# boqian-li/ETCH

Measured on AMD Instinct MI355X. Metric: scans/s (5k pts, eq-net + 50-iter SMPL fit), higher is better.
Workload: dtype f32 (matrix operands: 2 x fp16 planes per fp32 value, fp32 accumulate)

## Files before the change

### etch_amd/csrc/index_ops.hip

```cpp
#include "common.h"
#include <cmath>
#include <cstdio>

template <int WAVES>
__global__ void __launch_bounds__(WAVES * 64) ball_query_kernel(int n, int m, float radius2, int nsample,
                                                               const float* __restrict__ new_xyz,
                                                               const float* __restrict__ xyz, int* __restrict__ idx) {
    extern __shared__ __attribute__((aligned(16))) int smem_i[];
    const int lane = threadIdx.x & 63, wave = threadIdx.x >> 6;
    const int b = blockIdx.y;
    const float* X = xyz + (size_t)b * 3 * n;
    const float* Q = new_xyz + (size_t)b * 3 * m;
    int* row = smem_i + wave * nsample;
    for (int j = blockIdx.x * WAVES + wave; j < m; j += gridDim.x * WAVES) {
        const float qx = Q[j], qy = Q[m + j], qz = Q[2 * m + j];
        int cnt = 0;
        for (int k0 = 0; k0 < n && cnt < nsample; k0 += 64) {
            const int k = k0 + lane;
            bool in = false;
            if (k < n) {
                float d2 = etch_sqdist(qx, qy, qz, X[k], X[n + k], X[2 * n + k]);
                in = d2 < radius2;
            }
            const unsigned long long mask = __ballot(in);
// ... 455 lines not shown
        if (lane == 0) {
            for (int i = nsample - 1; i > 0; i--) {
                float tf = hd[0]; hd[0] = hd[i]; hd[i] = tf;
                int ti = hi[0]; hi[0] = hi[i]; hi[i] = ti;
                int root = 0, child = 1;
                while (child < i) {
                    if (child + 1 < i && hd[child + 1] > hd[child]) child++;
                    if (hd[root] > hd[child]) break;
                    const float tf2 = hd[root]; hd[root] = hd[child]; hd[child] = tf2;
                    const int ti2 = hi[root]; hi[root] = hi[child]; hi[child] = ti2;
                    root = child; child = root * 2 + 1;
                }
            }
        }
        __builtin_amdgcn_wave_barrier();
        for (int i = lane; i < nsample; i += 64) {
            idx[(size_t)q * nsample + i] = hi[i];
            const float d = hd[i];
            dist2[(size_t)q * nsample + i] = write_sqrt ? sqrtf(d) : d;
        }
        __builtin_amdgcn_wave_barrier();
}

__global__ void __launch_bounds__(KNNW_WAVES * 64) knn_wave_kernel(int nsample, int nseg, const float* __restrict__ xyz,
                                                                    const float* __restrict__ new_xyz, const int* __restrict__ offset,
                                                                    const int* __restrict__ new_offset, int m_total, int* __restrict__ idx,
                                                                    float* __restrict__ dist2, int write_sqrt) {
    extern __shared__ __attribute__((aligned(16))) float smem_f[];
    const int lane = threadIdx.x & 63, wave = threadIdx.x >> 6;
    float* hd = smem_f + wave * 2 * nsample;
    int* hi = (int*)(hd + nsample);
    float* cand_d = smem_f + KNNW_WAVES * 2 * nsample + wave * 128;
    int* cand_i = (int*)(cand_d + 64);
    for (int q = blockIdx.x * KNNW_WAVES + wave; q < m_total; q += gridDim.x * KNNW_WAVES) {
        int seg = 0;
        while (seg < nseg - 1 && q >= new_offset[seg]) ++seg;
        const int start = seg == 0 ? 0 : offset[seg - 1], end = offset[seg];
        if (nsample > 16) {
            knn_literal_query(q, start, end, nsample, lane, xyz, new_xyz, hd, hi, cand_d, cand_i, idx, dist2, write_sqrt);
            continue;
        }
        const float qx = new_xyz[(size_t)q * 3], qy = new_xyz[(size_t)q * 3 + 1], qz = new_xyz[(size_t)q * 3 + 2];
        float bd = 1e10f;
        int bi = start;
        float top = 1e10f;
        bool ambiguous = false;
        for (int k0 = start; k0 < end; k0 += 64) {
            const int k = k0 + lane;
            float d2 = 3e38f;
            if (k < end) d2 = etch_sqdist(qx, qy, qz, xyz[(size_t)k * 3], xyz[(size_t)k * 3 + 1], xyz[(size_t)k * 3 + 2]);
            unsigned long long mask = __ballot(d2 < top);
            while (mask) {
                const int e = __builtin_ctzll(mask);
                mask &= mask - 1ull;
                const float cd = __int_as_float(__builtin_amdgcn_readlane(__float_as_int(d2), e));
                if (cd < top) {
                    if (nsample > 1) {
                        const float t2 = __int_as_float(__builtin_amdgcn_readlane(__float_as_int(bd), nsample - 2));
                        if (t2 == top && __builtin_amdgcn_readlane(bi, nsample - 1) != __builtin_amdgcn_readlane(bi, nsample - 2)) ambiguous = true;
                    }
                    const int pos = __popcll(__ballot(lane < nsample && bd <= cd));
                    const float pd = __int_as_float(__builtin_amdgcn_update_dpp(0, __float_as_int(bd), 0x111, 0xf, 0xf, true));
                    const int pi = __builtin_amdgcn_update_dpp(0, bi, 0x111, 0xf, 0xf, true);
                    if (lane == pos) { bd = cd; bi = k0 + e; }
                    else if (lane > pos) { bd = pd; bi = pi; }
                    top = __int_as_float(__builtin_amdgcn_readlane(__float_as_int(bd), nsample - 1));
                }
            }
        }
        const float prev = __int_as_float(__builtin_amdgcn_update_dpp(0, __float_as_int(bd), 0x111, 0xf, 0xf, true));
        const int previ = __builtin_amdgcn_update_dpp(0, bi, 0x111, 0xf, 0xf, true);
        const bool tie = lane > 0 && lane < nsample && bd == prev && bi != previ;
        if (ambiguous || __ballot(tie) != 0ull) {
            knn_literal_query(q, start, end, nsample, lane, xyz, new_xyz, hd, hi, cand_d, cand_i, idx, dist2, write_sqrt);
            continue;
        }
        if (lane < nsample) {
            idx[(size_t)q * nsample + lane] = bi;
            dist2[(size_t)q * nsample + lane] = write_sqrt ? sqrtf(bd) : bd;
        }
    }
}

static inline int ilog2_floor_host(int v) { int b = 0; while ((1 << (b + 1)) <= v) ++b; return b; }

static int opt_n_threads_host(int work_size) {
    const int pow_2 = (int)(std::log((double)work_size) / std::log(2.0));
    int v = 1 << pow_2;
    if (v > 1024) v = 1024;
    if (v < 1) v = 1;
    return v;
}

static int g_fps_fast = 1;

static int launch_fps2(int nseg0, int nseg1, int n_max, const FpsProb& p0, const FpsProb& p1, hipStream_t st) {
    const int bs = opt_n_threads_host(n_max);
    const int bits = ilog2_floor_host(bs);
    const bool fits_lds = (size_t)3 * n_max * sizeof(float) <= 62 * 1024;
    const int nseg = nseg0 + nseg1;
#define FPS_CASE(T, P, R, C, COND)                                                                                     \
    if (n_max <= T * P && (COND)) {                                                                                    \
        const int use_lds = !C && fits_lds ? n_max : 0;                                                                \
        if (R && C && T == 1024 && bs == T && g_fps_fast)      \
            hipLaunchKernelGGL((fps_kernel<T, P, R, C, (R && C && T == 1024)>), dim3(nseg), dim3(T), (size_t)3 * use_lds * sizeof(float), st,   \
                               use_lds, p0, p1, nseg0, bs, bits);                                                      \
        else                                                                                                           \
            hipLaunchKernelGGL((fps_kernel<T, P, R, C>), dim3(nseg), dim3(T), (size_t)3 * use_lds * sizeof(float), st, \
                               use_lds, p0, p1, nseg0, bs, bits);                                                      \
        ETCH_RETURN_IF_LAUNCH_FAILED();                                                                                \
        return ETCH_OK;                                                                                                \
    }
    FPS_CASE(64, 1, true, false, true) FPS_CASE(64, 4, true, false, true) FPS_CASE(256, 2, true, false, true) FPS_CASE(256, 8, true, false, true)
    FPS_CASE(1024, 4, true, false, true) FPS_CASE(1024, 8, true, false, fits_lds) FPS_CASE(1024, 8, true, true, true)
    FPS_CASE(1024, 12, true, true, true) FPS_CASE(1024, 20, true, true, true) FPS_CASE(1024, 32, false, false, true)
#undef FPS_CASE
    return ETCH_EUNSUPPORTED;
}

static int launch_fps(int nseg, int n_max, const float* xyz, long cs, long ps, long bstride, int n_fixed, int m_fixed,
                      const int* offset, const int* new_offset, int skip_origin, int* idx, hipStream_t st) {
    const FpsProb p = {xyz, cs, ps, bstride, n_fixed, m_fixed, offset, new_offset, skip_origin, idx};
    return launch_fps2(nseg, 0, n_max, p, p, st);
}

static unsigned g_fps_spin_limit = 1u << 22;
static int g_fps_drop_group = -1;

static int launch_fps_split(int nseg, int n_max, int G, const float* xyz, long cs, long ps, long bstride, int n_fixed, int m_fixed, const int* offset,
                            const int* new_offset, int skip_origin, int* idx, void* workspace, hipStream_t st) {
    if (G < 2 || G > 8 || !workspace) return ETCH_EINVAL;
    const int bs = opt_n_threads_host(n_max);
    const int bits = ilog2_floor_host(bs);
    const int chunks = (n_max + 1023) / 1024, need = (chunks + G - 1) / G;
    const size_t bytes = 64 + (size_t)nseg * 2 * G * 64;
    hipError_t e = hipMemsetAsync(workspace, 0, bytes, st);
    if (e != hipSuccess) return (int)e;
#define FPS_SPLIT_CASE(P)                                                                                                                  \
    if (need <= P) {                                                                                                                       \
        hipLaunchKernelGGL((fps_split_kernel<P>), dim3(nseg * G), dim3(1024), 0, st, G, xyz, cs, ps, bstride, n_fixed, m_fixed, offset,    \
                           new_offset, bs, bits, skip_origin, g_fps_spin_limit, g_fps_drop_group, (unsigned long long*)workspace, idx);    \
        ETCH_RETURN_IF_LAUNCH_FAILED();                                                                                                    \
        return ETCH_OK;                                                                                                                    \
    }
    FPS_SPLIT_CASE(2) FPS_SPLIT_CASE(3) FPS_SPLIT_CASE(4) FPS_SPLIT_CASE(5) FPS_SPLIT_CASE(6) FPS_SPLIT_CASE(8)
#undef FPS_SPLIT_CASE
    return ETCH_EUNSUPPORTED;
}

extern "C" {

int etch_fps_split_workspace_bytes(int nseg, int G) { return nseg > 0 && G > 0 ? 64 + nseg * 2 * G * 64 : 64; }

int etch_furthest_point_sampling_split(int b, int n, int m, const float* xyz, int* idx, int G, void* workspace, void* stream) {
    if (b <= 0 || m <= 0) return ETCH_OK;
    if (n <= 0) return ETCH_EINVAL;
    return launch_fps_split(b, n, G, xyz, (long)n, 1, (long)3 * n, n, m, nullptr, nullptr, 1, idx, workspace, (hipStream_t)stream);
}

int etch_furthestsampling_split(int b, int n_max, const float* xyz, const int* offset, const int* new_offset, int* idx, int G, void* workspace,
                                void* stream) {
    if (b <= 0) return ETCH_OK;
    if (n_max <= 0) return ETCH_EINVAL;
    return launch_fps_split(b, n_max, G, xyz, 1, 3, 0, 0, 0, offset, new_offset, 0, idx, workspace, (hipStream_t)stream);
}

// ... 34 lines not shown

int etch_furthest_point_sampling(int b, int n, int m, const float* xyz, int* idx, void* stream) {
    if (b <= 0 || m <= 0) return ETCH_OK;
    if (n <= 0) return ETCH_EINVAL;
    return launch_fps(b, n, xyz, (long)n, 1, (long)3 * n, n, m, nullptr, nullptr, 1, idx, (hipStream_t)stream);
}

int etch_furthestsampling(int b, int n_max, const float* xyz, const int* offset, const int* new_offset, int* idx,
                          void* stream) {
    if (b <= 0) return ETCH_OK;
    if (n_max <= 0) return ETCH_EINVAL;
    return launch_fps(b, n_max, xyz, 1, 3, 0, 0, 0, offset, new_offset, 0, idx, (hipStream_t)stream);
}

int etch_fps_pair(int b, int n, int m, const float* xyz_b3n, int* idx_a, const float* xyz_packed, const int* offset, const int* new_offset, int* idx_b,
                  void* stream) {
    if (b <= 0) return ETCH_OK;
    if (n <= 0 || m <= 0 || !xyz_b3n || !xyz_packed || !offset || !new_offset || !idx_a || !idx_b) return ETCH_EINVAL;
    const FpsProb p0 = {xyz_b3n, (long)n, 1, (long)3 * n, n, m, nullptr, nullptr, 1, idx_a};
    const FpsProb p1 = {xyz_packed, 1, 3, 0, 0, 0, offset, new_offset, 0, idx_b};
    return launch_fps2(b, b, n, p0, p1, (hipStream_t)stream);
}

int etch_gather_points(int b, int c, int n, int m, const float* points, const int* idx, float* out, void* stream) {
    if (b <= 0 || m <= 0 || c <= 0) return ETCH_OK;
    int gx = (m + 255) / 256;
    if (gx > 8192) gx = 8192;
    hipLaunchKernelGGL(gather_points_kernel, dim3(gx, b), dim3(256), 0, (hipStream_t)stream, c, n, m, points, idx, out);
    ETCH_RETURN_IF_LAUNCH_FAILED();
    return ETCH_OK;
}

int etch_gather_points_backward(int b, int c, int n, int m, const float* grad_out, const int* idx, float* grad_points, void* stream) {
    if (b <= 0 || n <= 0 || c <= 0) return ETCH_OK;
    if (m < 0) return ETCH_EINVAL;
    int gx = (n + 255) / 256;
    if (gx > 8192) gx = 8192;
    hipLaunchKernelGGL(gather_points_backward_kernel, dim3(gx, b), dim3(256), 0, (hipStream_t)stream, c, n, m, grad_out, idx, grad_points);
    ETCH_RETURN_IF_LAUNCH_FAILED();
    return ETCH_OK;
}

int etch_knnquery(int b, int m_max, int m_total, int nsample, const float* xyz, const float* new_xyz, const int* offset,
                  const int* new_offset, int* idx, float* dist, int write_sqrt, void* stream) {
    if (b <= 0 || m_max <= 0) return ETCH_OK;
    if (nsample <= 0) return ETCH_EINVAL;
    if (m_total > 0) {
        if (nsample > 100) return ETCH_EUNSUPPORTED;
        const size_t lds = (size_t)(KNNW_WAVES * 2 * nsample + KNNW_WAVES * 128) * 4;
        long blocks = ((long)m_total + KNNW_WAVES - 1) / KNNW_WAVES;
        if (blocks > 256 * 64) blocks = 256 * 64;
        hipLaunchKernelGGL(knn_wave_kernel, dim3((unsigned)blocks), dim3(KNNW_WAVES * 64), lds, (hipStream_t)stream, nsample, b, xyz,
                           new_xyz, offset, new_offset, m_total, idx, dist, write_sqrt);
        ETCH_RETURN_IF_LAUNCH_FAILED();
        return ETCH_OK;
    }
    if (nsample > 28) return ETCH_EUNSUPPORTED;
    const size_t lds = (size_t)(3 * KNN_TILE + 2 * nsample * KNN_THREADS) * 4;
    hipLaunchKernelGGL(knn_kernel, dim3((m_max + KNN_THREADS - 1) / KNN_THREADS, b), dim3(KNN_THREADS), lds,
                       (hipStream_t)stream, nsample, xyz, new_xyz, offset, new_offset, idx, dist, write_sqrt);
    ETCH_RETURN_IF_LAUNCH_FAILED();
    return ETCH_OK;
}

int etch_knnquery_dev_bounded(int m, int nsample, int nseg, const float* xyz, const float* new_xyz, const int* offset, const int* new_offset,
                              int* idx, float* dist, int write_sqrt, void* stream) {
    if (m <= 0) return ETCH_OK;
    if (nsample <= 0 || nseg <= 0) return ETCH_EINVAL;
    if (nsample > 100) return ETCH_EUNSUPPORTED;
    const size_t lds = (size_t)(KNNW_WAVES * 2 * nsample + KNNW_WAVES * 128) * 4;
    long blocks = ((long)m + KNNW_WAVES - 1) / KNNW_WAVES;
    if (blocks > 256 * 64) blocks = 256 * 64;
    hipLaunchKernelGGL(knn_wave_kernel, dim3((unsigned)blocks), dim3(KNNW_WAVES * 64), lds, (hipStream_t)stream, nsample, nseg, xyz,
                       new_xyz, offset, new_offset, m, idx, dist, write_sqrt);
    ETCH_RETURN_IF_LAUNCH_FAILED();
    return ETCH_OK;
}

int etch_knnquery_dev(int m, int nsample, const float* xyz, const float* new_xyz, const int* offset, const int* new_offset, int* idx,
                      float* dist, int write_sqrt, void* stream) {
    return etch_knnquery_dev_bounded(m, nsample, 0x7fffffff, xyz, new_xyz, offset, new_offset, idx, dist, write_sqrt, stream);
}

static void report_launcher(const char* name, int rc) {
    if (rc != ETCH_OK) fprintf(stderr, "Error: %s failed (%d%s%s)\n", name, rc, rc > 0 ? ": " : "", rc > 0 ? hipGetErrorString((hipError_t)rc) : "");
}

void knnquery_cuda_launcher(int m, int nsample, const float* xyz, const float* new_xyz, const int* offset, const int* new_offset, int* idx,
                            float* dist2) {
    report_launcher("knnquery_cuda_launcher", etch_knnquery_dev(m, nsample, xyz, new_xyz, offset, new_offset, idx, dist2, 0, nullptr));
}

void furthestsampling_cuda_launcher(int b, int n, const float* xyz, const int* offset, const int* new_offset, float* tmp, int* idx) {
    (void)tmp;
    report_launcher("furthestsampling_cuda_launcher", etch_furthestsampling(b, n, xyz, offset, new_offset, idx, nullptr));
}

void ball_query_cuda_launcher(int b, int n, int m, float radius, int nsample, const float* new_xyz, const float* xyz, int* idx) {
    report_launcher("ball_query_cuda_launcher", etch_ball_query(b, n, m, radius, nsample, new_xyz, xyz, idx, nullptr));
}

void furthest_point_sampling_cuda_launcher(int b, int n, int m, const float* dataset, float* temp, int* idxs) {
    (void)temp;
    report_launcher("furthest_point_sampling_cuda_launcher", etch_furthest_point_sampling(b, n, m, dataset, idxs, nullptr));
}

void gather_points_forward_cuda_launcher(int b, int c, int n, int m, const float* points, const int* idx, float* out) {
    report_launcher("gather_points_forward_cuda_launcher", etch_gather_points(b, c, n, m, points, idx, out, nullptr));
}

void gather_points_backward_cuda_launcher(int b, int c, int n, int m, const float* grad_out, const int* idx, float* grad_points) {
    report_launcher("gather_points_backward_cuda_launcher", etch_gather_points_backward(b, c, n, m, grad_out, idx, grad_points, nullptr));
}

}

__device__ __forceinline__ unsigned etch_spread10(unsigned v) {
    v = (v | (v << 16)) & 0x030000FFu;
    v = (v | (v << 8)) & 0x0300F00Fu;
    v = (v | (v << 4)) & 0x030C30C3u;
    v = (v | (v << 2)) & 0x09249249u;
    return v;
}

__global__ void __launch_bounds__(1024) spatial_order_kernel(int n, int np2, const float* __restrict__ xyz, int* __restrict__ order) {
    extern __shared__ __attribute__((aligned(16))) unsigned long long keys[];
    __shared__ float red[6][16];
    const int b = blockIdx.x, tid = threadIdx.x, lane = tid & 63, wave = tid >> 6;
    const float* X = xyz + (size_t)b * 3 * n;
    float lo[3] = {INFINITY, INFINITY, INFINITY}, hi[3] = {-INFINITY, -INFINITY, -INFINITY};
    for (int i = tid; i < n; i += 1024)
#pragma unroll
        for (int a = 0; a < 3; ++a) { const float v = X[(size_t)a * n + i]; lo[a] = fminf(lo[a], v); hi[a] = fmaxf(hi[a], v); }
#pragma unroll
    for (int a = 0; a < 3; ++a) {
        float l = lo[a], h = hi[a];
        for (int o = 32; o > 0; o >>= 1) { l = fminf(l, __shfl_xor(l, o)); h = fmaxf(h, __shfl_xor(h, o)); }
        if (lane == 0) { red[a][wave] = l; red[3 + a][wave] = h; }
    }
    __syncthreads();
    float mn[3], sc[3];
#pragma unroll
    for (int a = 0; a < 3; ++a) {
        float l = red[a][0], h = red[3 + a][0];
        for (int w = 1; w < 16; ++w) { l = fminf(l, red[a][w]); h = fmaxf(h, red[3 + a][w]); }
        mn[a] = l;
        sc[a] = h > l ? 1023.0f / (h - l) : 0.f;
    }
    for (int i = tid; i < np2; i += 1024) {
        unsigned long long k = ~0ull;
        if (i < n) {
            unsigned q[3];
#pragma unroll
            for (int a = 0; a < 3; ++a) {
                const float t = (X[(size_t)a * n + i] - mn[a]) * sc[a];
                q[a] = (unsigned)fminf(fmaxf(t, 0.f), 1023.f);
            }
            const unsigned m = etch_spread10(q[0]) | (etch_spread10(q[1]) << 1) | (etch_spread10(q[2]) << 2);
            k = ((unsigned long long)m << 32) | (unsigned)i;
        }
        keys[i] = k;
    }
    __syncthreads();
    for (int size = 2; size <= np2; size <<= 1)
        for (int stride = size >> 1; stride > 0; stride >>= 1) {
            for (int i = tid; i < (np2 >> 1); i += 1024) {
// ... 90 lines not shown
```

### etch_amd/models/pointops.py

```python
import torch

from .. import ops

_knn_cache = None


def host_offsets(o):
    v = getattr(o, "_etch_host", None)
    if v is None or getattr(o, "_etch_host_version", -1) != o._version:
        v = [int(t) for t in o.tolist()]
        set_host_offsets(o, v)
    return v


def set_host_offsets(o, values):
    o._etch_host = list(values)
    o._etch_host_version = o._version
    return o


_offset_tensors = {}


def offsets_tensor(values, device):
    device = torch.device(device)
    key = (tuple(int(v) for v in values), device.type, device.index if device.index is not None else torch.cuda.current_device())
    t = _offset_tensors.get(key)
    if t is None:
        t = set_host_offsets(torch.tensor(list(key[0]), dtype=torch.int32, device=device), key[0])
        torch.cuda.current_stream(device).synchronize()
        if len(_offset_tensors) > 256:
            _offset_tensors.clear()
        _offset_tensors[key] = t
    return t


class knn_scope:

    def __enter__(self):
        global _knn_cache
        self._prev = _knn_cache
        if _knn_cache is None:
            _knn_cache = {}
        return self

    def __exit__(self, *a):
        global _knn_cache
        _knn_cache = self._prev


def _memo(key, keep, fn):
    if _knn_cache is None:
        return fn()
    hit = _knn_cache.get(key)
    if hit is None:
        hit = (fn(), keep)
        _knn_cache[key] = hit
    return hit[0]


def make_offsets(values, device, like=None):
    return offsets_tensor(values, device)


def furthestsampling(xyz, offset, new_offset):
    oh, noh = host_offsets(offset), host_offsets(new_offset)
    return _memo(("fps", xyz.data_ptr(), tuple(oh), tuple(noh)), (xyz,), lambda: ops.furthestsampling(xyz, offset, new_offset, oh, noh))


def gather_rows(x, idx):
    return _memo(("rows", x.data_ptr(), idx.data_ptr()), (x, idx), lambda: ops.gather_rows(x, idx))


def knnquery(nsample, xyz, new_xyz, offset, new_offset):
    if new_xyz is None:
        new_xyz = xyz
    oh, noh = host_offsets(offset), host_offsets(new_offset)
    return _memo(("knn", nsample, xyz.data_ptr(), new_xyz.data_ptr(), tuple(oh), tuple(noh)), (xyz, new_xyz),
                 lambda: ops.knnquery(nsample, xyz, new_xyz, offset, new_offset, noh))


def queryandgroup(nsample, xyz, new_xyz, feat, idx, offset, new_offset, use_xyz=True):
    if new_xyz is None:
        new_xyz = xyz
    if idx is None:
        idx = knnquery(nsample, xyz, new_xyz, offset, new_offset)[0]
    m, c = new_xyz.shape[0], feat.shape[1]
    g = ops.pt_group(xyz, new_xyz, feat, idx).view(m, nsample, 3 + c)
    return g if use_xyz else g[:, :, 3:]


def interpolation(xyz, new_xyz, feat, offset, new_offset, k=3, add_to=None):
    assert k == 3
    r = knnquery(k, xyz, new_xyz, offset, new_offset)
    idx, dist = r[0], r[1]
    if add_to is None:
        add_to = torch.zeros((new_xyz.shape[0], feat.shape[1]), dtype=torch.float32, device=feat.device)
    return ops.pt_interp_add(add_to, feat, idx, dist)
```

### etch_amd/models/pointtransformer_seg.py

```python
import os

import torch
import torch.nn as nn

from .. import ops
from ..vgtk_so3conv import _Derived
from . import pointops


def fold_bn(bn):
    s = bn.weight.detach() / torch.sqrt(bn.running_var + bn.eps)
    return s.contiguous(), (bn.bias.detach() - bn.running_mean * s).contiguous()



def downsampled_offsets(oh, stride):
    n_o, count, prev = [], 0, 0
    for i, end in enumerate(oh):
        m = (end - prev) // stride
        if m <= 0:
            raise ValueError(f"scan {i} has {end - prev} points at a stride-{stride} TransitionDown: too few for the five-level "
                             f"Point-Transformer nets (a scan needs at least 256 points)")
        count += m
        n_o.append(count)
# ... 245 lines not shown
        return x1


class PointTransformer_confidence(_PointTransformerBase):

    def __init__(self, block, blocks, c=6, k=13):
        super().__init__()
        self.c, self.k = c, k
        planes = [128, 128, 256, 256, 512]
        self._build(block, blocks, c, planes)
        self.cls = nn.Sequential(nn.Conv1d(planes[0], planes[0], 1), nn.BatchNorm1d(planes[0]), nn.ReLU(), nn.Conv1d(planes[0], k, 1))
        self.confi = nn.Sequential(nn.Conv1d(planes[0], planes[0] * k, 1), nn.ReLU(), nn.Conv1d(planes[0] * k, 1 * k, 1, groups=k))
        self._d, self._dw = _Derived(), _Derived()

    def forward(self, pxo):
        p0, x0, o0 = pxo
        B = o0.shape[0]
        N = p0.shape[0] // B
        with pointops.knn_scope():
            x1 = self._unet(pxo)
        s, t = self._d.get([self.cls[1].weight, self.cls[1].bias, self.cls[1].running_mean, self.cls[1].running_var], lambda: fold_bn(self.cls[1]))
        h = ops.linear(x1, self.cls[0].weight.detach().view(self.cls[0].out_channels, -1), bias=self.cls[0].bias.detach(), scale=s, shift=t, act="relu")
        logits = ops.linear(h, self.cls[3].weight.detach().view(self.k, -1), bias=self.cls[3].bias.detach())
        w0 = self.confi[0].weight.detach().view(self.confi[0].out_channels, -1)
        b0 = self.confi[0].bias.detach()
        w2 = self.confi[2].weight.detach().view(self.k, -1).contiguous()
        b2 = self.confi[2].bias.detach()
        wp = self._dw.get([self.confi[0].weight], lambda: ops.permute_weight_frag_grouped(w0.contiguous(), w2.shape[1]))
        conf_k = ops.linear_relu_dot(x1, w0, b0, w2.view(-1), b2, self.k, wp=wp)
        conf = ops.softmax_dot(logits, conf_k)
        return logits.view(B, N, self.k), conf.view(B, N, 1)


class PointTransformer_magnitude(_PointTransformerBase):

    def __init__(self, block, blocks, c=6, k=1):
        super().__init__()
        self.c = c
        assert k == 1, "Please check output dim of PointTransformer_magnitude"
        planes = [64, 128, 256, 256, 512]
        self._build(block, blocks, c, planes)
        self.final_layer = nn.Sequential(nn.Linear(planes[0], planes[0]), nn.BatchNorm1d(planes[0]), nn.ReLU(inplace=True), nn.Linear(planes[0], 1))
        self._d = _Derived()

    def forward(self, pxo):
        p0, x0, o0 = pxo
        B = o0.shape[0]
        N = p0.shape[0] // B
        with pointops.knn_scope():
            x1 = self._unet(pxo)
        fl = self.final_layer
        s, t = self._d.get([fl[1].weight, fl[1].bias, fl[1].running_mean, fl[1].running_var], lambda: fold_bn(fl[1]))
        h = ops.linear(x1, fl[0].weight.detach(), bias=fl[0].bias.detach(), scale=s, shift=t, act="relu")
        y = ops.linear(h, fl[3].weight.detach(), bias=fl[3].bias.detach())
        return y.view(B, N, 1)


def get_pointtransformer_confidence(**kwargs):
    return PointTransformer_confidence(PointTransformerBlock, [2, 3, 4, 6, 3], **kwargs)


def get_pointtransformer_magnitude(**kwargs):
    return PointTransformer_magnitude(PointTransformerBlock, [2, 3, 4, 6, 3], **kwargs)


def prefetch_indices(p0, o0, strides=(1, 4, 4, 4, 4), nsamples=(8, 16, 16, 16, 16)):
    made = []
    levels = []
    p, o = p0, o0
    for li in range(5):
        if strides[li] != 1:
            oh = pointops.host_offsets(o)
            n_o = downsampled_offsets(oh, strides[li])
            n_o_t = pointops.make_offsets(n_o, p.device, like=(o, strides[li]))
            idx = pointops.furthestsampling(p, o, n_o_t)
            n_p = pointops.gather_rows(p, idx)
            made += [idx, n_p, n_o_t] + list(pointops.knnquery(nsamples[li], p, n_p, o, n_o_t))
            p, o = n_p, n_o_t
        made += list(pointops.knnquery(nsamples[li], p, p, o, o))
        levels.append((p, o))
    for li in range(3, -1, -1):
        (pf, of), (pc, oc) = levels[li], levels[li + 1]
        made += list(pointops.knnquery(3, pc, pf, oc, of))
    return made
```

### etch_amd/ops.py

```python
import ctypes
import math
import os

import torch

from . import _lib

_c_int, _c_float, _vp = ctypes.c_int, ctypes.c_float, ctypes.c_void_p


_raw_stream = getattr(torch._C, "_cuda_getCurrentRawStream", None)


def _stream():
    if _raw_stream is not None:
        return _vp(_raw_stream(torch.cuda.current_device()))
    return _vp(torch.cuda.current_stream().cuda_stream)


def _ptr(t):
    return _vp(t.data_ptr())


def _need(t, dtype, name):
# ... 31 lines not shown
        return g if g >= 2 else 1
    return 1


def _fps_split_ws(nseg, G, device):
    ws = torch.empty((_lib.lib().etch_fps_split_workspace_bytes(nseg, G),), dtype=torch.uint8, device=device)
    return ws


def fps_split_failed(idx):
    ws = getattr(idx, "_etch_split_ws", None)
    if ws is None:
        return False
    out = ctypes.c_int(0)
    _lib.check(_lib.lib().etch_fps_split_failed(_ptr(ws), ctypes.byref(out), _stream()), "etch_fps_split_failed")
    return bool(out.value)


def _fps_split_checked(idx, split):
    if split is None and fps_split_failed(idx):
        raise _lib.EtchHipError("split FPS gave up (a workgroup of a scan never arrived): rerun with ETCH_FPS_SPLIT unset (one workgroup per scan)")
    return idx


_FPS_READY = {}


def fps_pair(xyz_b3n, m, xyz_packed, offset, new_offset, new_offset_host):
    _need(xyz_b3n, torch.float32, "xyz_b3n"), _need(xyz_packed, torch.float32, "xyz_packed")
    _need(offset, torch.int32, "offset"), _need(new_offset, torch.int32, "new_offset")
    b, _, n = xyz_b3n.shape
    assert xyz_packed.shape == (b * n, 3)
    idx_a = torch.zeros((b, m), dtype=torch.int32, device=xyz_b3n.device)
    idx_b = torch.zeros((int(new_offset_host[-1]),), dtype=torch.int32, device=xyz_b3n.device)
    _lib.check(_lib.lib().etch_fps_pair(b, n, int(m), _ptr(xyz_b3n), _ptr(idx_a), _ptr(xyz_packed), _ptr(offset), _ptr(new_offset), _ptr(idx_b), _stream()),
               "etch_fps_pair")
    return idx_a, idx_b


def furthest_point_sampling(xyz, m, split=None):
    _need(xyz, torch.float32, "xyz")
    b, _, n = xyz.shape
    ready = _FPS_READY.pop(("vgtk", xyz.data_ptr(), int(m)), None) if _FPS_READY else None
    if ready is not None:
        return ready
    idx = torch.zeros((b, m), dtype=torch.int32, device=xyz.device)
    G = fps_split_default(b, n, xyz.device) if split is None else int(split)
    if G >= 2:
        ws = _fps_split_ws(b, G, xyz.device)
        _lib.check(_lib.lib().etch_furthest_point_sampling_split(b, n, int(m), _ptr(xyz), _ptr(idx), G, _ptr(ws), _stream()),
                   "etch_furthest_point_sampling_split")
        idx._etch_split_ws = ws
        return _fps_split_checked(idx, split)
    _lib.check(_lib.lib().etch_furthest_point_sampling(b, n, int(m), _ptr(xyz), _ptr(idx), _stream()), "etch_furthest_point_sampling")
    return idx


def gather_points_forward(points, idx):
    _need(points, torch.float32, "points"), _need(idx, torch.int32, "idx")
    b, c, n = points.shape
    m = idx.shape[1]
    out = torch.empty((b, c, m), dtype=torch.float32, device=points.device)
    _lib.check(_lib.lib().etch_gather_points(b, c, n, m, _ptr(points), _ptr(idx), _ptr(out), _stream()), "etch_gather_points")
    return out


def gather_points_backward(grad_out, idx, npoint):
    _need(grad_out, torch.float32, "grad_out"), _need(idx, torch.int32, "idx")
    b, c, m = grad_out.shape
    out = torch.empty((b, c, int(npoint)), dtype=torch.float32, device=grad_out.device)
    _lib.check(_lib.lib().etch_gather_points_backward(b, c, int(npoint), m, _ptr(grad_out), _ptr(idx), _ptr(out), _stream()),
               "etch_gather_points_backward")
    return out


def _seg_max(offset_host):
    prev, mx = 0, 0
    for v in offset_host:
        mx = max(mx, int(v) - prev)
        prev = int(v)
    return mx


def knnquery(nsample, xyz, new_xyz, offset, new_offset, new_offset_host=None, sqrt=True, wave_kernel=True):
    if new_xyz is None:
        new_xyz = xyz
    _need(xyz, torch.float32, "xyz"), _need(new_xyz, torch.float32, "new_xyz")
    _need(offset, torch.int32, "offset"), _need(new_offset, torch.int32, "new_offset")
    if new_offset_host is None:
        new_offset_host = new_offset.tolist()
    m = new_xyz.shape[0]
    idx = torch.empty((m, nsample), dtype=torch.int32, device=xyz.device)
    dist = torch.empty((m, nsample), dtype=torch.float32, device=xyz.device)
    _lib.check(_lib.lib().etch_knnquery(len(new_offset_host), _seg_max(new_offset_host), int(m) if wave_kernel else 0, int(nsample), _ptr(xyz), _ptr(new_xyz),
                                        _ptr(offset), _ptr(new_offset), _ptr(idx), _ptr(dist), 1 if sqrt else 0, _stream()),
               "etch_knnquery")
    return idx, dist


def furthestsampling(xyz, offset, new_offset, offset_host=None, new_offset_host=None, split=None):
    _need(xyz, torch.float32, "xyz"), _need(offset, torch.int32, "offset"), _need(new_offset, torch.int32, "new_offset")
    if offset_host is None:
        offset_host = offset.tolist()
    if new_offset_host is None:
        new_offset_host = new_offset.tolist()
    ready = _FPS_READY.pop(("pointops", xyz.data_ptr(), new_offset.data_ptr()), None) if _FPS_READY else None
    if ready is not None:
        return ready
    idx = torch.zeros((int(new_offset_host[-1]),), dtype=torch.int32, device=xyz.device)
    nseg, n_max = len(offset_host), _seg_max(offset_host)
    G = fps_split_default(nseg, n_max, xyz.device) if split is None else int(split)
    if G >= 2:
        ws = _fps_split_ws(nseg, G, xyz.device)
        _lib.check(_lib.lib().etch_furthestsampling_split(nseg, n_max, _ptr(xyz), _ptr(offset), _ptr(new_offset), _ptr(idx), G, _ptr(ws), _stream()),
                   "etch_furthestsampling_split")
        idx._etch_split_ws = ws
        return _fps_split_checked(idx, split)
    _lib.check(_lib.lib().etch_furthestsampling(nseg, n_max, _ptr(xyz), _ptr(offset), _ptr(new_offset), _ptr(idx), _stream()), "etch_furthestsampling")
    return idx


_c_long = ctypes.c_long
ACT = {None: 0, "none": 0, "relu": 1, "leaky_relu": 2}


def _optptr(t):
    return _vp(0) if t is None else _ptr(t)


def linear(x, weight, bias=None, scale=None, shift=None, act=None, res=None, res_mode=0, row_idx=None, grp=1, p_in=0, p_out=1,
           rows=None, out=None):
    _need(weight, torch.float32, "weight")
    if x.dtype != torch.float32 or not x.is_cuda:
        raise _lib.EtchHipError("x must be a float32 CUDA(HIP) tensor")
    K = x.shape[-1]
    assert x.stride(-1) == 1 and weight.shape[1] == K, (x.shape, weight.shape)
    x2 = x if x.dim() == 2 else x.reshape(-1, K)
    ldx = x2.stride(0) if x2.shape[0] > 1 else K
    R = x2.shape[0] if rows is None else rows
    O = weight.shape[0]
    if out is None:
        out = torch.empty((R, O), dtype=torch.float32, device=x.device)
    ldr = res.stride(0) if res is not None and res.dim() == 2 and res.shape[0] > 1 else O
    _lib.check(_lib.lib().etch_linear(int(R), int(K), int(O), _ptr(x2), _c_long(ldx), _optptr(row_idx), int(grp), int(p_in), int(p_out),
                                      _ptr(weight), _c_long(weight.stride(0)), _optptr(bias), _optptr(scale), _optptr(shift),
                                      ACT[act], _optptr(res), _c_long(ldr), int(res_mode), _ptr(out), _c_long(out.stride(0)), _stream()),
               "etch_linear")
    return out


def permute_weight_frag(w2):
    O, K = w2.shape
    assert O % 16 == 0 and K % 16 == 0
    return w2.reshape(O // 16, 16, K // 16, 4, 4).permute(2, 0, 3, 1, 4).contiguous().reshape(-1)


def permute_weight_frag32(w2):
    O, K = w2.shape
    assert O % 32 == 0 and K % 8 == 0
    return w2.reshape(O // 32, 32, K // 8, 2, 4).permute(2, 0, 3, 1, 4).contiguous().reshape(-1)


def inter_weight_frag(W, cin, ks=24):
    return permute_weight_frag(W[:, _inter_contraction_cols(cin, ks, W.device)].contiguous())


_CONTRACTION_COLS = {}


def _inter_contraction_cols(cin, ks, device):
    key = (cin, ks, str(device))
    if key not in _CONTRACTION_COLS:
        _CONTRACTION_COLS[key] = _inter_contraction_cols_build(cin, ks, device)
    return _CONTRACTION_COLS[key]


# ... 985 lines not shown
```

### include/etch_hip.h

```cpp
#ifndef ETCH_HIP_H
#define ETCH_HIP_H

#ifdef __cplusplus
extern "C" {
#endif


int etch_ball_query(int b, int n, int m, float radius, int nsample, const float* new_xyz, const float* xyz,
                    int* idx, void* stream);

int etch_furthest_point_sampling(int b, int n, int m, const float* xyz, int* idx, void* stream);

int etch_fps_split_workspace_bytes(int nseg, int G);
int etch_furthest_point_sampling_split(int b, int n, int m, const float* xyz, int* idx, int G, void* workspace, void* stream);
int etch_furthestsampling_split(int b, int n_max, const float* xyz, const int* offset, const int* new_offset, int* idx, int G, void* workspace,
                                void* stream);
int etch_fps_split_failed(const void* workspace, int* failed, void* stream);
int etch_fps_split_debug(unsigned spin_limit, int drop_group);
int etch_fps_fast(int enable);

int etch_gather_points(int b, int c, int n, int m, const float* points, const int* idx, float* out, void* stream);

int etch_gather_points_backward(int b, int c, int n, int m, const float* grad_out, const int* idx, float* grad_points, void* stream);


int etch_knnquery(int b, int m_max, int m_total, int nsample, const float* xyz, const float* new_xyz, const int* offset,
                  const int* new_offset, int* idx, float* dist, int write_sqrt, void* stream);

int etch_furthestsampling(int b, int n_max, const float* xyz, const int* offset, const int* new_offset, int* idx,
                          void* stream);
int etch_fps_pair(int b, int n, int m, const float* xyz_b3n, int* idx_a, const float* xyz_packed, const int* offset, const int* new_offset, int* idx_b,
                  void* stream);

int etch_knnquery_dev(int m, int nsample, const float* xyz, const float* new_xyz, const int* offset, const int* new_offset, int* idx,
                      float* dist, int write_sqrt, void* stream);
int etch_knnquery_dev_bounded(int m, int nsample, int nseg, const float* xyz, const float* new_xyz, const int* offset, const int* new_offset,
                              int* idx, float* dist, int write_sqrt, void* stream);


void knnquery_cuda_launcher(int m, int nsample, const float* xyz, const float* new_xyz, const int* offset, const int* new_offset, int* idx,
                            float* dist2);
void furthestsampling_cuda_launcher(int b, int n, const float* xyz, const int* offset, const int* new_offset, float* tmp, int* idx);
void ball_query_cuda_launcher(int b, int n, int m, float radius, int nsample, const float* new_xyz, const float* xyz, int* idx);
void furthest_point_sampling_cuda_launcher(int b, int n, int m, const float* dataset, float* temp, int* idxs);
void gather_points_forward_cuda_launcher(int b, int c, int n, int m, const float* points, const int* idx, float* out);
void gather_points_backward_cuda_launcher(int b, int c, int n, int m, const float* grad_out, const int* idx, float* grad_points);


int etch_linear(int R, int K, int O, const float* X, long ldx, const int* row_idx, int grp, int p_in, int p_out,
                const float* W, long ldw, const float* bias, const float* scale, const float* shift, int act,
                const float* res, long ldr, int res_mode, float* Y, long ldy, void* stream);


int etch_inter_so3conv(int b, int cin, int cout, int p1, int p2, int nn, float sigma, const float* xyz,
                       const float* new_xyz, const int* ball_idx, const float* feats, const float* rk, const float* W,
                       const float* Wp, const float* bias, float* out, void* stream);

int etch_inter_so3conv_ordered(int b, int cin, int cout, int p1, int p2, int nn, float sigma, const float* xyz, const float* new_xyz,
                               const int* ball_idx, const float* feats, const float* rk, const float* W, const float* Wp,
                               const float* bias, float* out, const int* order, double* stat_part, void* stream);

#ifdef ETCH_BUILD_EXPERIMENTS
int etch_inter_so3conv32(int b, int cin, int cout, int p1, int p2, int nn, float sigma, const float* xyz, const float* new_xyz,
                         const int* ball_idx, const float* feats, const float* rk, const float* Wp32, const float* bias, float* out,
                         const int* order, double* stat_part, void* stream);
#endif

int etch_inter_so3conv_split(int b, int cin, int cout, int p1, int p2, int nn, float sigma, const float* xyz, const float* new_xyz,
                             const int* ball_idx, const float* feats, const float* rk, const void* Wq, const float* bias, float* out,
                             const int* order, double* stat_part, void* stream);

int etch_inter_so3conv_planes_supported(int cin, int cout, int nn);

#ifdef ETCH_BUILD_EXPERIMENTS
int etch_inter_so3conv_planes(int b, int cin, int cout, int p1, int p2, int nn, float sigma, const float* xyz, const float* new_xyz,
                              const int* ball_idx, const void* feats_planes, const float* rk, const void* Wq, const float* bias, float* out,
                              const int* order, double* stat_part, void* stream);
int etch_inter_so3conv_planes32(int b, int cin, int cout, int p1, int p2, int nn, float sigma, const float* xyz, const float* new_xyz,
                                const int* ball_idx, const void* feats_planes, const float* rk, const void* Wq32, const float* bias, float* out,
                                const int* order, double* stat_part, void* stream);
#endif

int etch_inter_kpoint_operand(float sigma, const float* rk, void* kq, void* stream);
int etch_inter_so3conv_planes_kq(int b, int cin, int cout, int p1, int p2, int nn, float sigma, const float* xyz, const float* new_xyz,
                                 const int* ball_idx, const void* feats_planes, const void* kq, const void* Wq32, const float* wsc, const float* fsc,
                                 const float* bias, float* out, const int* order, double* stat_part, void* stream);

int etch_split2_planes_f16(long rows, int C, const float* x, void* planes, void* stream);
int etch_split2_planes_f16_scaled(int b, long rows, int C, const float* x, void* mx, void* planes, float* fsc, void* stream);

int etch_split3_planes(long rows, int C, const float* x, void* planes, void* stream);

int etch_instnorm_from_partials(int b, int nparts, int C, int count, const double* partial, float* mean, float* rstd, void* stream);

int etch_spatial_order(int b, int n, const float* xyz, int* order, void* stream);

int etch_intra_so3conv(int b, int c, int cout, int p, const float* X, const float* mean, const float* rstd,
                       const int* intra_idx, const float* Wp, const float* bias, float* Y, void* stream);
int etch_intra_so3conv_stats(int b, int c, int cout, int p, const float* X, const float* mean, const float* rstd,
                             const int* intra_idx, const float* Wp, const float* bias, float* Y, double* stat_part, void* stream);
int etch_intra_so3conv32(int b, int c, int cout, int p, const float* X, const float* mean, const float* rstd, const int* intra_idx,
                         const float* Wp32, const float* bias, float* Y, double* stat_part, void* stream);

int etch_intra_so3conv_split(int b, int c, int cout, int p, const float* X, const float* mean, const float* rstd, const int* intra_idx,
                             const void* Wq, const float* bias, float* Y, double* stat_part, void* stream);

int etch_intra_so3conv_f16(int b, int c, int cout, int p, const float* X, const float* mean, const float* rstd, const int* intra_idx,
                           const void* Wqh, const float* wsc, const float* bias, float* Y, double* stat_part, void* stream);

int etch_instnorm_stats(int b, int rows, int C, const float* x, double* workspace, float* mean, float* rstd, void* stream);
int etch_instnorm_stats_workspace_bytes(int b, int C);

int etch_instnorm_act_add(int b, int rows, int C, const float* x1, const float* m1, const float* r1, const float* x2,
                          const float* m2, const float* r2, float* out, void* stream);
int etch_instnorm_act_add_planes(int b, int rows, int C, const float* x1, const float* m1, const float* r1, const float* x2,
                                 const float* m2, const float* r2, float* out, void* planes, void* stream);
int etch_instnorm_act_add_planes_f16(int b, int rows, int C, const float* x1, const float* m1, const float* r1, const float* x2,
                                     const float* m2, const float* r2, float* out, void* planes, void* stream);
int etch_instnorm_act_add_k1_planes_f16(int b, int rows, int C, const float* x1, const float* m1, const float* r1, const float* f, const float* slope,
                                        const float* offset, float* out, void* planes, void* stream);
// ... 206 lines not shown
```

Measured before the change: 1015.

## Add axis-sorted sweep KNN with pruning and exact fallback

Adds a per-segment kernel that sorts points along the axis with the largest extent using an in-LDS bitonic sort. A sweep kernel then binary-searches each query's position in that order and expands left and right in 64-point chunks, stopping once the axis gap exceeds the current k-th distance. This replaces the brute-force scan over all segment points for small k. Ties and non-finite inputs fall back to the literal query. The sort result is memoized per point cloud, and the extra sort kernel adds overhead when segments are small.

```diff
diff --git a/etch_amd/csrc/index_ops.hip b/etch_amd/csrc/index_ops.hip
--- a/etch_amd/csrc/index_ops.hip
+++ b/etch_amd/csrc/index_ops.hip
@@ -561,6 +561,239 @@
     }
 }
 
+#define KNN_SORT_MAX 16384
+__device__ __forceinline__ unsigned etch_float_order_u32(float v) {
+    const unsigned u = __float_as_uint(v);
+    return (u & 0x80000000u) ? ~u : (u | 0x80000000u);
+}
+
+__global__ void __launch_bounds__(1024) knn_sort_kernel(int cap, const float* __restrict__ xyz, const int* __restrict__ offset,
+                                                        float4* __restrict__ rec, int* __restrict__ axis) {
+    extern __shared__ __attribute__((aligned(16))) unsigned long long skeys[];
+    __shared__ float red[6][16];
+    const int seg = blockIdx.x, tid = threadIdx.x, lane = tid & 63, wave = tid >> 6;
+    const int start = seg == 0 ? 0 : offset[seg - 1], n = offset[seg] - start;
+    if (n <= 0 || n > cap) {
+        if (tid == 0) axis[seg] = -1;
+        return;
+    }
+    int np2 = 2;
+    while (np2 < n) np2 <<= 1;
+    const float* X = xyz + (size_t)start * 3;
+    float lo[3] = {INFINITY, INFINITY, INFINITY}, hi[3] = {-INFINITY, -INFINITY, -INFINITY};
+    int bad = 0;
+    for (int i = tid; i < n; i += 1024)
+#pragma unroll
+        for (int a = 0; a < 3; ++a) {
+            const float v = X[(size_t)i * 3 + a];
+            bad |= !(fabsf(v) <= 3.402823466e38f);
+            lo[a] = fminf(lo[a], v); hi[a] = fmaxf(hi[a], v);
+        }
+#pragma unroll
+    for (int a = 0; a < 3; ++a) {
+        float l = lo[a], h = hi[a];
+        for (int o = 32; o > 0; o >>= 1) { l = fminf(l, __shfl_xor(l, o)); h = fmaxf(h, __shfl_xor(h, o)); }
+        if (lane == 0) { red[a][wave] = l; red[3 + a][wave] = h; }
+    }
+    if (__syncthreads_or(bad)) {
+        if (tid == 0) axis[seg] = -1;
+        return;
+    }
+    int ax = 0;
+    float best = -1.f;
+#pragma unroll
+    for (int a = 0; a < 3; ++a) {
+        float l = red[a][0], h = red[3 + a][0];
+        for (int w = 1; w < 16; ++w) { l = fminf(l, red[a][w]); h = fmaxf(h, red[3 + a][w]); }
+        const float ext = h - l;
+        if (ext > best) { best = ext; ax = a; }
+    }
+    for (int i = tid; i < np2; i += 1024)
+        skeys[i] = i < n ? ((unsigned long long)etch_float_order_u32(X[(size_t)i * 3 + ax]) << 32) | (unsigned)i : ~0ull;
+    __syncthreads();
+    for (int size = 2; size <= np2; size <<= 1)
+        for (int stride = size >> 1; stride > 0; stride >>= 1) {
+            for (int i = tid; i < (np2 >> 1); i += 1024) {
+                const int lowi = ((i / stride) * (stride << 1)) + (i % stride), highi = lowi + stride;
+                const bool up = ((lowi & size) == 0);
+                const unsigned long long x = skeys[lowi], y = skeys[highi];
+                if ((x > y) == up) { skeys[lowi] = y; skeys[highi] = x; }
+            }
+            __syncthreads();
+        }
+    for (int i = tid; i < n; i += 1024) {
+        const int j = (int)(unsigned)(skeys[i] & 0xFFFFFFFFull);
+        rec[(size_t)start + i] = make_float4(X[(size_t)j * 3], X[(size_t)j * 3 + 1], X[(size_t)j * 3 + 2], __int_as_float(start + j));
+    }
+    if (tid == 0) axis[seg] = ax;
+}
+
+__device__ __forceinline__ void knn_list_insert(float cd, int ci, int nsample, int lane, float& bd, int& bi, float& top, bool& ambiguous) {
+    if (nsample > 1) {
+        const float t2 = __int_as_float(__builtin_amdgcn_readlane(__float_as_int(bd), nsample - 2));
+        if (t2 == top && __builtin_amdgcn_readlane(bi, nsample - 1) != __builtin_amdgcn_readlane(bi, nsample - 2)) ambiguous = true;
+    }
+    const int pos = __popcll(__ballot(lane < nsample && bd <= cd));
+    const float pd = __int_as_float(__builtin_amdgcn_update_dpp(0, __float_as_int(bd), 0x111, 0xf, 0xf, true));
+    const int pi = __builtin_amdgcn_update_dpp(0, bi, 0x111, 0xf, 0xf, true);
+    if (lane == pos) { bd = cd; bi = ci; }
+    else if (lane > pos) { bd = pd; bi = pi; }
+    top = __int_as_float(__builtin_amdgcn_readlane(__float_as_int(bd), nsample - 1));
+}
+
+__global__ void __launch_bounds__(KNNW_WAVES * 64) knn_sweep_kernel(int nsample, int nseg, const float* __restrict__ xyz,
+                                                                     const float4* __restrict__ rec, const int* __restrict__ axis,
+                                                                     const float* __restrict__ new_xyz, const int* __restrict__ offset,
+                                                                     const int* __restrict__ new_offset, int m_total, int* __restrict__ idx,
+                                                                     float* __restrict__ dist2, int write_sqrt, unsigned* __restrict__ fallback_count) {
+    extern __shared__ __attribute__((aligned(16))) float smem_f[];
+    const int lane = threadIdx.x & 63, wave = threadIdx.x >> 6;
+    float* hd = smem_f + wave * 2 * nsample;
+    int* hi = (int*)(hd + nsample);
+    float* cand_d = smem_f + KNNW_WAVES * 2 * nsample + wave * 128;
+    int* cand_i = (int*)(cand_d + 64);
+    int vo = 0, va = -1;
+    if (lane < nseg) { vo = offset[lane]; va = axis[lane]; }
+    for (int q = blockIdx.x * KNNW_WAVES + wave; q < m_total; q += gridDim.x * KNNW_WAVES) {
+        int seg = 0;
+        for (int s0 = 0; s0 < nseg - 1; s0 += 64) {
+            const int s = s0 + lane;
+            const int c = __popcll(__ballot(s < nseg - 1 && q >= new_offset[s]));
+            seg += c;
+            if (c < 64) break;
+        }
+        int start, end, ax;
+        if (seg < 64) {
+            end = __builtin_amdgcn_readlane(vo, seg);
+            start = seg == 0 ? 0 : __builtin_amdgcn_readlane(vo, seg - 1);
+            ax = __builtin_amdgcn_readlane(va, seg);
+        } else {
+            start = offset[seg - 1]; end = offset[seg]; ax = axis[seg];
+        }
+        const int n = end - start;
+        const float qx = new_xyz[(size_t)q * 3], qy = new_xyz[(size_t)q * 3 + 1], qz = new_xyz[(size_t)q * 3 + 2];
+        const bool finite_q = fabsf(qx) <= 3.402823466e38f && fabsf(qy) <= 3.402823466e38f && fabsf(qz) <= 3.402823466e38f;
+        float bd = 1e10f;
+        int bi = start;
+        bool literal = ax < 0 || !finite_q;
+        if (!literal) {
+            const float qa = ax == 0 ? qx : (ax == 1 ? qy : qz);
+            const float* ra = (const float*)(rec + start) + ax;
+            int lo = 0, hi_ = n;
+            while (hi_ - lo > 32) {
+                const int step = (hi_ - lo + 63) >> 6;
+                const int p = lo + lane * step;
+                const int c = __popcll(__ballot(p < hi_ && ra[(size_t)p * 4] < qa));
+                const int nh = lo + c * step;
+                if (c > 0) lo = lo + (c - 1) * step + 1;
+                if (nh < hi_) hi_ = nh;
+            }
+            const int pos = lo + ((hi_ - lo) >> 1);
+            float top = 1e10f;
+            bool ambiguous = false;
+            float rej = -1.f;
+            int L = pos - 32;
+            if (L > n - 64) L = n - 64;
+            if (L < 0) L = 0;
+            int R = L + 64 < n ? L + 64 : n;
+            float fl, fr;
+            float4 rr = make_float4(0.f, 0.f, 0.f, 0.f), rl = rr;
+            {
+                const int bl0 = L - 64 > 0 ? L - 64 : 0;
+                if (R + lane < n) rr = rec[(size_t)start + R + lane];
+                if (lane < L - bl0) rl = rec[(size_t)start + bl0 + lane];
+            }
+            bool fetched = true;
+            {
+                const bool valid = L + lane < R;
+                float4 r = make_float4(0.f, 0.f, 0.f, 0.f);
+                if (valid) r = rec[(size_t)start + L + lane];
+                const float d2 = valid ? etch_sqdist(qx, qy, qz, r.x, r.y, r.z) : 3e38f;
+                const int gi = valid ? __float_as_int(r.w) : start;
+                const float da = qa - (ax == 0 ? r.x : (ax == 1 ? r.y : r.z));
+                const float da2 = da * da;
+                fl = __int_as_float(__builtin_amdgcn_readlane(__float_as_int(da2), 0));
+                fr = __shfl(da2, R - L - 1);
+                const unsigned me = __float_as_uint(d2);
+                cand_d[lane] = d2;
+                __builtin_amdgcn_wave_barrier();
+                int rank = 0;
+#pragma unroll 2
+                for (int j = 0; j < 16; ++j) {
+                    const uint4 o = ((const uint4*)cand_d)[j];
+                    rank += (o.x < me ? 1 : 0) + (o.y < me ? 1 : 0) + (o.z < me ? 1 : 0) + (o.w < me ? 1 : 0);
+                }
+                cand_i[rank] = lane;
+                __builtin_amdgcn_wave_barrier();
+                if (__ballot(((volatile int*)cand_i)[rank] != lane) != 0ull) {
+                    rank = 0;
+#pragma unroll 1
+                    for (int j = 0; j < 64; ++j) {
+                        const unsigned o = __float_as_uint(cand_d[j]);
+                        rank += (o < me || (o == me && j < lane)) ? 1 : 0;
+                    }
+                }
+                if (rank < nsample) { hd[rank] = d2; hi[rank] = gi; }
+                __builtin_amdgcn_wave_barrier();
+                if (lane < nsample) {
+                    const float sd = hd[lane];
+                    if (sd < 1e10f) { bd = sd; bi = hi[lane]; }
+                }
+                __builtin_amdgcn_wave_barrier();
+                top = __int_as_float(__builtin_amdgcn_readlane(__float_as_int(bd), nsample - 1));
+                if (__ballot(valid && d2 == top && gi != __builtin_amdgcn_readlane(bi, nsample - 1)) != 0ull) rej = top;
+            }
+            bool go_r = R < n && fr <= top, go_l = L > 0 && fl <= top;
+            while (go_r || go_l) {
+                const int cr = go_r ? (n - R < 64 ? n - R : 64) : 0;
+                const int bl = L - 64 > 0 ? L - 64 : 0;
+                const int cl = go_l ? L - bl : 0;
+                if (!fetched) {
+                    if (lane < cr) rr = rec[(size_t)start + R + lane];
+                    if (lane < cl) rl = rec[(size_t)start + bl + lane];
+                }
+                fetched = false;
+#pragma unroll
+                for (int side = 0; side < 2; ++side) {
+                    const int cnt = side == 0 ? cr : cl;
+                    if (cnt == 0) continue;
+                    const float4 r = side == 0 ? rr : rl;
+                    const bool valid = lane < cnt;
+                    const float d2 = valid ? etch_sqdist(qx, qy, qz, r.x, r.y, r.z) : 3e38f;
+                    const int gi = valid ? __float_as_int(r.w) : start;
+                    const float da = qa - (ax == 0 ? r.x : (ax == 1 ? r.y : r.z));
+                    const float da2 = da * da;
+                    if (side == 0) { fr = __shfl(da2, cnt - 1); R += cnt; }
+                    else { fl = __int_as_float(__builtin_amdgcn_readlane(__float_as_int(da2), 0)); L = bl; }
+                    unsigned long long mask = __ballot(d2 < top);
+                    while (mask) {
+                        const int e = __builtin_ctzll(mask);
+                        mask &= mask - 1ull;
+                        const float cd = __int_as_float(__builtin_amdgcn_readlane(__float_as_int(d2), e));
+                        if (cd < top) knn_list_insert(cd, __builtin_amdgcn_readlane(gi, e), nsample, lane, bd, bi, top, ambiguous);
+                    }
+                    if (__ballot(valid && d2 == top && gi != __builtin_amdgcn_readlane(bi, nsample - 1)) != 0ull) rej = top;
+                }
+                go_r = R < n && fr <= top;
+                go_l = L > 0 && fl <= top;
+            }
+            const float prev = __int_as_float(__builtin_amdgcn_update_dpp(0, __float_as_int(bd), 0x111, 0xf, 0xf, true));
+            const int previ = __builtin_amdgcn_update_dpp(0, bi, 0x111, 0xf, 0xf, true);
+            const bool tie = lane > 0 && lane < nsample && bd == prev && bi != previ;
+            literal = ambiguous || rej == top || __ballot(tie) != 0ull;
+        }
+        if (literal) {
+            knn_literal_query(q, start, end, nsample, lane, xyz, new_xyz, hd, hi, cand_d, cand_i, idx, dist2, write_sqrt);
+            if (fallback_count && lane == 0) atomicAdd(fallback_count, 1u);
+            continue;
+        }
+        if (lane < nsample) {
+            idx[(size_t)q * nsample + lane] = bi;
+            dist2[(size_t)q * nsample + lane] = write_sqrt ? sqrtf(bd) : bd;
+        }
+    }
+}
+
 static inline int ilog2_floor_host(int v) { int b = 0; while ((1 << (b + 1)) <= v) ++b; return b; }
 
 static int opt_n_threads_host(int work_size) {
@@ -761,6 +994,36 @@
     return etch_knnquery_dev_bounded(m, nsample, 0x7fffffff, xyz, new_xyz, offset, new_offset, idx, dist, write_sqrt, stream);
 }
 
+int etch_knn_sort(int nseg, int n_max, const float* xyz, const int* offset, void* rec, int* axis, void* stream) {
+    if (nseg <= 0) return ETCH_OK;
+    if (n_max <= 0) return ETCH_EINVAL;
+    int np2 = 2;
+    while (np2 < n_max && np2 < KNN_SORT_MAX) np2 <<= 1;
+    const int cap = n_max < np2 ? n_max : np2;
+    const size_t lds = (size_t)np2 * sizeof(unsigned long long);
+    if (lds > 64 * 1024) {
+        hipError_t e = hipFuncSetAttribute((const void*)knn_sort_kernel, hipFuncAttributeMaxDynamicSharedMemorySize, (int)lds);
+        if (e != hipSuccess) return (int)e;
+    }
+    hipLaunchKernelGGL(knn_sort_kernel, dim3((unsigned)nseg), dim3(1024), lds, (hipStream_t)stream, cap, xyz, offset, (float4*)rec, axis);
+    ETCH_RETURN_IF_LAUNCH_FAILED();
+    return ETCH_OK;
+}
+
+int etch_knn_sweep(int m, int nsample, int nseg, const float* xyz, const void* rec, const int* axis, const float* new_xyz, const int* offset,
+                   const int* new_offset, int* idx, float* dist, int write_sqrt, unsigned* fallback_count, void* stream) {
+    if (m <= 0) return ETCH_OK;
+    if (nsample <= 0 || nseg <= 0) return ETCH_EINVAL;
+    if (nsample > 16) return ETCH_EUNSUPPORTED;
+    const size_t lds = (size_t)(KNNW_WAVES * 2 * nsample + KNNW_WAVES * 128) * 4;
+    long blocks = ((long)m + KNNW_WAVES - 1) / KNNW_WAVES;
+    if (blocks > 256 * 64) blocks = 256 * 64;
+    hipLaunchKernelGGL(knn_sweep_kernel, dim3((unsigned)blocks), dim3(KNNW_WAVES * 64), lds, (hipStream_t)stream, nsample, nseg, xyz,
+                       (const float4*)rec, axis, new_xyz, offset, new_offset, m, idx, dist, write_sqrt, fallback_count);
+    ETCH_RETURN_IF_LAUNCH_FAILED();
+    return ETCH_OK;
+}
+
 static void report_launcher(const char* name, int rc) {
     if (rc != ETCH_OK) fprintf(stderr, "Error: %s failed (%d%s%s)\n", name, rc, rc > 0 ? ": " : "", rc > 0 ? hipGetErrorString((hipError_t)rc) : "");
 }
diff --git a/etch_amd/models/pointops.py b/etch_amd/models/pointops.py
--- a/etch_amd/models/pointops.py
+++ b/etch_amd/models/pointops.py
@@ -76,8 +76,18 @@
     if new_xyz is None:
         new_xyz = xyz
     oh, noh = host_offsets(offset), host_offsets(new_offset)
-    return _memo(("knn", nsample, xyz.data_ptr(), new_xyz.data_ptr(), tuple(oh), tuple(noh)), (xyz, new_xyz),
-                 lambda: ops.knnquery(nsample, xyz, new_xyz, offset, new_offset, noh))
+
+    def run():
+        if not ops.knn_sweep_applies(nsample, oh):
+            return ops.knnquery(nsample, xyz, new_xyz, offset, new_offset, noh, pruned=False)
+        srt = _memo(("knnsort", xyz.data_ptr(), tuple(oh)), (xyz,), lambda: ops.knn_sort(xyz, offset, oh))
+        return ops.knnquery(nsample, xyz, new_xyz, offset, new_offset, noh, pruned=True, offset_host=oh, sorted_points=srt)
+
+    return _memo(("knn", nsample, xyz.data_ptr(), new_xyz.data_ptr(), tuple(oh), tuple(noh)), (xyz, new_xyz), run)
+
+
+def knn_sort_workspaces():
+    return [t for key, (val, _) in (_knn_cache or {}).items() if key[0] == "knnsort" for t in val]
 
 
 def queryandgroup(nsample, xyz, new_xyz, feat, idx, offset, new_offset, use_xyz=True):
diff --git a/etch_amd/models/pointtransformer_seg.py b/etch_amd/models/pointtransformer_seg.py
--- a/etch_amd/models/pointtransformer_seg.py
+++ b/etch_amd/models/pointtransformer_seg.py
@@ -351,4 +351,5 @@
     for li in range(3, -1, -1):
         (pf, of), (pc, oc) = levels[li], levels[li + 1]
         made += list(pointops.knnquery(3, pc, pf, oc, of))
+    made += pointops.knn_sort_workspaces()
     return made
diff --git a/etch_amd/ops.py b/etch_amd/ops.py
--- a/etch_amd/ops.py
+++ b/etch_amd/ops.py
@@ -137,16 +137,63 @@
     return mx
 
 
-def knnquery(nsample, xyz, new_xyz, offset, new_offset, new_offset_host=None, sqrt=True, wave_kernel=True):
+KNN_SWEEP_MAX_NSAMPLE = 16
+KNN_SWEEP_MAX_POINTS = 16384
+KNN_SWEEP_MIN_POINTS = 256
+
+
+def _seg_sizes(offset_host):
+    prev, out = 0, []
+    for v in offset_host:
+        out.append(int(v) - prev)
+        prev = int(v)
+    return out
+
+
+def knn_sweep_applies(nsample, offset_host):
+    sizes = _seg_sizes(offset_host)
+    return nsample <= KNN_SWEEP_MAX_NSAMPLE and len(sizes) > 0 and min(sizes) >= KNN_SWEEP_MIN_POINTS and max(sizes) <= KNN_SWEEP_MAX_POINTS
+
+
+def knn_sort(xyz, offset, offset_host=None):
+    _need(xyz, torch.float32, "xyz"), _need(offset, torch.int32, "offset")
+    if offset_host is None:
+        offset_host = offset.tolist()
+    rec = torch.empty((xyz.shape[0], 4), dtype=torch.float32, device=xyz.device)
+    axis = torch.empty((len(offset_host),), dtype=torch.int32, device=xyz.device)
+    if xyz.shape[0] > 0:
+        _lib.check(_lib.lib().etch_knn_sort(len(offset_host), max(1, _seg_max(offset_host)), _ptr(xyz), _ptr(offset), _ptr(rec), _ptr(axis), _stream()),
+                   "etch_knn_sort")
+    return rec, axis
+
+
+def knnquery(nsample, xyz, new_xyz, offset, new_offset, new_offset_host=None, sqrt=True, wave_kernel=True, pruned=None, offset_host=None,
+             sorted_points=None, fallback_counter=None):
     if new_xyz is None:
         new_xyz = xyz
     _need(xyz, torch.float32, "xyz"), _need(new_xyz, torch.float32, "new_xyz")
     _need(offset, torch.int32, "offset"), _need(new_offset, torch.int32, "new_offset")
+    need_offset = pruned is None and wave_kernel and offset_host is None and nsample <= KNN_SWEEP_MAX_NSAMPLE
+    if need_offset and new_offset_host is None and offset is not new_offset:
+        both = torch.cat([offset, new_offset]).tolist()
+        offset_host, new_offset_host = both[:offset.shape[0]], both[offset.shape[0]:]
     if new_offset_host is None:
         new_offset_host = new_offset.tolist()
+    if need_offset and offset_host is None:
+        offset_host = new_offset_host if offset is new_offset else offset.tolist()
     m = new_xyz.shape[0]
     idx = torch.empty((m, nsample), dtype=torch.int32, device=xyz.device)
     dist = torch.empty((m, nsample), dtype=torch.float32, device=xyz.device)
+    if pruned is None and wave_kernel:
+        pruned = offset_host is not None and knn_sweep_applies(nsample, offset_host)
+    if pruned and wave_kernel:
+        if m > 0:
+            rec, axis = sorted_points if sorted_points is not None else knn_sort(xyz, offset, offset_host)
+            _lib.check(_lib.lib().etch_knn_sweep(int(m), int(nsample), len(new_offset_host), _ptr(xyz), _ptr(rec), _ptr(axis), _ptr(new_xyz), _ptr(offset),
+                                                 _ptr(new_offset), _ptr(idx), _ptr(dist), 1 if sqrt else 0,
+                                                 _ptr(fallback_counter) if fallback_counter is not None else None, _stream()),
+                       "etch_knn_sweep")
+        return idx, dist
     _lib.check(_lib.lib().etch_knnquery(len(new_offset_host), _seg_max(new_offset_host), int(m) if wave_kernel else 0, int(nsample), _ptr(xyz), _ptr(new_xyz),
                                         _ptr(offset), _ptr(new_offset), _ptr(idx), _ptr(dist), 1 if sqrt else 0, _stream()),
                "etch_knnquery")
diff --git a/include/etch_hip.h b/include/etch_hip.h
--- a/include/etch_hip.h
+++ b/include/etch_hip.h
@@ -36,6 +36,10 @@
                       float* dist, int write_sqrt, void* stream);
 int etch_knnquery_dev_bounded(int m, int nsample, int nseg, const float* xyz, const float* new_xyz, const int* offset, const int* new_offset,
                               int* idx, float* dist, int write_sqrt, void* stream);
+
+int etch_knn_sort(int nseg, int n_max, const float* xyz, const int* offset, void* rec, int* axis, void* stream);
+int etch_knn_sweep(int m, int nsample, int nseg, const float* xyz, const void* rec, const int* axis, const float* new_xyz, const int* offset,
+                   const int* new_offset, int* idx, float* dist, int write_sqrt, unsigned* fallback_count, void* stream);
 
 
 void knnquery_cuda_launcher(int m, int nsample, const float* xyz, const float* new_xyz, const int* offset, const int* new_offset, int* idx,
```

Result: faster. 1044 (median of 6 runs) (+2.8%).
